# google/dynamic-video-depth

Measured on AMD Instinct MI355X. Metric: train iters/s (depth+sceneflow step) at 384x672, 48 pairs; warp+loss HBM GB/s, higher is better.
Workload: dtype f32 (storage and accumulation fp32; conv / MLP contractions on v_mfma_f32_32x32x16_f16: every fp32 operand, scaled by a power of two from its tensor's max, is split into two fp16 terms (22 bits) and a product is three partial products; <= 4e-6 of max|y| against float64, the bound the 3-term bf16 / 6

## Files before the change

### dynamic-video-depth_amd/dvd_hip/_lib.py

```python
import ctypes
import os
import threading

from . import build as _build

c_float_p = ctypes.c_void_p
c_size_t = ctypes.c_size_t
c_int = ctypes.c_int
c_float = ctypes.c_float
c_void_p = ctypes.c_void_p

DVD_OK, DVD_EINVAL, DVD_EHIP, DVD_ENOSPC = 0, -1, -2, -3
ABI_VERSION = 8


class Cameras(ctypes.Structure):
    _fields_ = [(n, c_void_p) for n in ('R_1', 'R_2', 'R_1_T', 'R_2_T', 't_1', 't_2', 'K', 'K_inv')]


class WarpCfg(ctypes.Structure):
    _fields_ = [('B', c_int), ('H', c_int), ('W', c_int), ('midas_mask', c_int), ('crit_l2', c_int),
                ('disp_mode', c_int), ('loss_on_sf', c_int), ('flow_mul', c_float), ('disp_mul', c_float)]


# ... 60 lines not shown
    'dvd_sf_mlp_gstash_bytes': (c_size_t, [c_longlong]),
    'dvd_sf_mlp_pack': (c_int, [ctypes.POINTER(MlpDesc), ctypes.POINTER(PtrArr6), ctypes.POINTER(PtrArr6), c_void_p,
                                c_void_p]),
    'dvd_sf_mlp_fwd': (c_int, [ctypes.POINTER(MlpDesc), c_void_p, c_void_p, c_void_p, c_float, c_float, c_longlong,
                               c_int, c_void_p, c_void_p, c_void_p, c_void_p, c_void_p]),
    'dvd_sf_mlp_bwd_dx': (c_int, [ctypes.POINTER(MlpDesc), c_void_p, c_void_p, c_float, c_void_p, c_float, c_void_p,
                                  c_void_p, c_void_p, c_longlong, c_int, c_void_p, c_void_p, c_void_p, c_void_p,
                                  c_void_p]),
    'dvd_mul_mask': (c_int, [c_void_p, c_void_p, c_void_p, c_int, c_int, c_longlong, c_void_p]),
    'dvd_scale_add': (c_int, [c_void_p, c_void_p, c_float, c_void_p, c_void_p, c_longlong, c_void_p]),
    'dvd_subsample2_fwd': (c_int, [c_void_p, c_void_p, c_int, c_longlong, c_int, c_int, c_void_p]),
    'dvd_subsample2_bwd': (c_int, [c_void_p, c_void_p, c_int, c_longlong, c_int, c_int, c_void_p]),
    'dvd_avgpool_fwd': (c_int, [c_void_p, c_void_p, c_int, c_longlong] + [c_int] * 5 + [c_void_p]),
    'dvd_avgpool_bwd': (c_int, [c_void_p, c_void_p, c_int, c_longlong] + [c_int] * 5 + [c_void_p]),
    'dvd_depth_tail_fwd': (c_int, [c_void_p, c_void_p, c_longlong, c_void_p]),
    'dvd_depth_tail_bwd': (c_int, [c_void_p, c_void_p, c_void_p, c_longlong, c_void_p]),
    'dvd_acc_reg_workspace_bytes': (c_size_t, []),
    'dvd_acc_reg': (c_int, [c_void_p, c_void_p, c_float, c_void_p, c_void_p, c_void_p, c_int, c_longlong, c_void_p]),
    'dvd_adam_step': (c_int, [c_void_p, c_void_p, c_float, c_void_p, c_void_p, c_void_p, c_void_p, c_longlong, c_float,
                              c_float, c_float, c_float, c_int, c_void_p]),
    'dvd_warp_surfaces': (c_int, [c_void_p, c_void_p, c_void_p, c_void_p, ctypes.POINTER(Cameras),
                                  ctypes.POINTER(Surfaces), c_int, c_int, c_int, c_void_p]),
    'dvd_warp_surfaces_bwd': (c_int, [c_void_p, c_void_p, c_void_p, c_void_p, ctypes.POINTER(Cameras),
                                      ctypes.POINTER(Surfaces), c_void_p, c_void_p, c_void_p, c_int, c_int, c_int, c_void_p]),
    'dvd_flow_warp_fwd': (c_int, [c_void_p, c_void_p, c_void_p, c_int, c_int, c_int, c_int, c_void_p]),
    'dvd_flow_warp_bwd': (c_int, [c_void_p, c_void_p, c_void_p, c_int, c_int, c_int, c_int, c_void_p]),
    'dvd_bnrelu_fwd': (c_int, [c_void_p] * 6 + [c_float, c_void_p, c_int, c_int, c_int, c_int, c_void_p]),
    'dvd_bnrelu_bwd_workspace_bytes': (c_size_t, [c_int, c_int, c_int]),
    'dvd_bnrelu_bwd': (c_int, [c_void_p] * 6 + [c_float] + [c_void_p] * 5 + [c_size_t, c_int, c_int, c_int, c_int,
                                                                           c_void_p, c_void_p]),
    'dvd_upsample_bilinear_fwd': (c_int, [c_void_p, c_void_p, c_longlong, c_int, c_int, c_int, c_int, c_int, c_void_p]),
    'dvd_upsample_bilinear_bwd': (c_int, [c_void_p, c_void_p, c_longlong, c_int, c_int, c_int, c_int, c_int, c_void_p]),
    'dvd_gconv3x3_c8_fwd': (c_int, [c_void_p, c_void_p, c_void_p, c_int, c_int, c_int, c_int, c_void_p]),
    'dvd_gconv3x3_c8_bwd_data': (c_int, [c_void_p, c_void_p, c_void_p, c_int, c_int, c_int, c_int, c_void_p]),
    'dvd_gconv3x3_c8_wgrad_workspace_bytes': (c_size_t, [c_int, c_int, c_int, c_int]),
    'dvd_gconv3x3_c8_bwd_weight': (c_int, [c_void_p, c_void_p, c_void_p, c_int, c_void_p, c_size_t, c_int, c_int, c_int,
                                           c_int, c_void_p]),
    'dvd_gconv3x3_c32_workspace_bytes': (c_size_t, [c_int, c_int, c_int, c_int]),
    'dvd_gconv3x3_c32_fwd': (c_int, [c_void_p, c_void_p, c_void_p, c_void_p, c_size_t, c_int, c_int, c_int, c_int,
                                     c_void_p]),
    'dvd_gconv3x3_c32_bwd_data': (c_int, [c_void_p, c_void_p, c_void_p, c_void_p, c_size_t, c_int, c_int, c_int, c_int,
                                          c_void_p]),
    'dvd_gconv3x3_c32_bwd_weight': (c_int, [c_void_p, c_void_p, c_void_p, c_int, c_void_p, c_size_t, c_int, c_int,
                                            c_int, c_int, c_void_p]),
    'dvd_xconv_packed_bytes': (c_size_t, [c_int] * 5),
    'dvd_xconv_pack': (c_int, [c_void_p, c_void_p, c_int, c_int, c_int, c_int, c_int, c_void_p]),
    'dvd_xconv_pack_table_bytes': (c_size_t, [c_int]),
    'dvd_xconv_pack_many': (c_int, [c_void_p, c_int, c_void_p, c_size_t, c_int, c_void_p]),
    'dvd_amax': (c_int, [c_void_p, ctypes.c_longlong, c_void_p, c_void_p]),
    'dvd_chansum_workspace_bytes': (c_size_t, [c_int, c_int]),
    'dvd_chansum': (c_int, [c_void_p, c_int, c_int, ctypes.c_longlong, c_void_p, c_void_p, c_void_p, c_size_t, c_void_p]),
    'dvd_xconv_fwd': (c_int, [c_void_p] * 6 + [ctypes.POINTER(BnParams), c_void_p, c_void_p] + [c_int] * 8 + [c_void_p]),
    'dvd_xconv_select': (c_int, [c_int]),
    'dvd_xconv_pack_scaled': (c_int, [c_void_p, c_void_p, c_int, c_int, c_int, c_int, c_int, c_void_p, c_void_p, c_float,
                                      c_void_p]),
    'dvd_convbn_finalize': (c_int, [c_void_p] * 6 + [c_float, c_void_p, c_int, c_int, c_void_p, c_void_p, c_void_p]),
    'dvd_xwgrad3_workspace_bytes': (c_size_t, [c_int] * 6),
    'dvd_xwgrad1s_workspace_bytes': (c_size_t, [c_int] * 5),
    'dvd_xwgrad_select': (c_int, [c_int]),
    'dvd_sf_mlp_select': (c_int, [c_int]),
    'dvd_xwgradk_workspace_bytes': (c_size_t, [c_int] * 6),
    'dvd_xwgradk': (c_int, [c_void_p] * 6 + [c_size_t] + [c_int] * 7 + [c_void_p]),
    'dvd_xwgrad1s': (c_int, [c_void_p] * 6 + [c_size_t] + [c_int] * 6 + [c_void_p]),
    'dvd_xwgrad1s_rowsum': (c_int, [c_void_p] * 7 + [c_size_t] + [c_int] * 6 + [c_void_p]),
    'dvd_xwgrad3_rowsum': (c_int, [c_void_p] * 7 + [c_size_t] + [c_int] * 7 + [c_void_p]),
    'dvd_xwgrad_rowsum_in_kernel': (c_int, [c_int] * 7),
    'dvd_xwgrad3': (c_int, [c_void_p] * 6 + [c_size_t] + [c_int] * 7 + [c_void_p]),
    'dvd_xwgrad_workspace_bytes': (c_size_t, [c_int] * 6),
    'dvd_xwgrad': (c_int, [c_void_p] * 4 + [c_size_t] + [c_int] * 7 + [c_void_p]),
    'dvd_flow_consistency_mask': (c_int, [c_void_p, c_void_p, c_void_p, c_int, c_int, c_int, c_void_p]),
    'dvd_sf_mlp_bwd_dw': (c_int, [ctypes.POINTER(MlpDesc), c_void_p, c_void_p, c_longlong, ctypes.POINTER(PtrArr5),
                                  ctypes.POINTER(PtrArr5), c_void_p]),
    'dvd_xconv_fwd_h': (c_int, [c_void_p] * 5 + [ctypes.POINTER(BnParams), c_void_p, c_void_p] + [c_int] * 9 + [c_void_p]),
    'dvd_xwgrad3_h': (c_int, [c_void_p] * 5 + [c_size_t] + [c_int] * 7 + [c_void_p]),
    'dvd_xwgrad1s_h': (c_int, [c_void_p] * 5 + [c_size_t] + [c_int] * 6 + [c_void_p]),
    'dvd_xwgradk_h': (c_int, [c_void_p] * 5 + [c_size_t] + [c_int] * 7 + [c_void_p]),
    'dvd_bnrelu_fwd_t': (c_int, [c_void_p] * 6 + [c_float, c_void_p, c_int, c_int, c_int, c_int, c_int, c_void_p]),
    'dvd_bnrelu_bwd_t': (c_int, [c_void_p] * 6 + [c_float] + [c_void_p] * 5 + [c_size_t, c_int, c_void_p, c_int, c_int, c_int,
                                                                             c_int, c_void_p, c_void_p]),
    'dvd_bnrelu_fwd_m': (c_int, [c_void_p] * 6 + [c_float, c_void_p, c_int, c_int, c_int, c_int, c_int, c_void_p, c_void_p]),
    'dvd_bnrelu_bwd_m': (c_int, [c_void_p] * 6 + [c_float] + [c_void_p] * 5 + [c_size_t, c_int, c_void_p, c_int, c_int, c_int,
                                                                             c_int, c_void_p, c_void_p, c_void_p]),
    'dvd_upsample_bilinear_fwd_t': (c_int, [c_void_p, c_void_p, c_int, c_longlong, c_int, c_int, c_int, c_int, c_int, c_void_p]),
    'dvd_upsample_bilinear_bwd_t': (c_int, [c_void_p, c_void_p, c_int, c_longlong, c_int, c_int, c_int, c_int, c_int, c_void_p]),
    'dvd_bicubic_fwd': (c_int, [c_void_p, c_void_p, c_longlong, c_int, c_int, c_int, c_int, c_void_p, c_void_p, c_int, c_void_p]),
    'dvd_bicubic_bwd_workspace_bytes': (c_size_t, [c_longlong, c_int, c_int, c_int, c_int]),
    'dvd_bicubic_bwd': (c_int, [c_void_p, c_void_p, c_longlong, c_int, c_int, c_int, c_int, c_void_p, c_size_t, c_void_p]),
    'dvd_gconv3x3_c8_fwd_t': (c_int, [c_void_p, c_void_p, c_void_p, c_int, c_int, c_int, c_int, c_int, c_void_p]),
    'dvd_gconv3x3_c8_bwd_data_t': (c_int, [c_void_p, c_void_p, c_void_p, c_int, c_int, c_int, c_int, c_int, c_void_p]),
    'dvd_gconv3x3_c8_bwd_weight_t': (c_int, [c_void_p, c_void_p, c_void_p, c_int, c_void_p, c_size_t, c_int, c_void_p, c_int,
                                             c_int, c_int, c_int, c_void_p]),
    'dvd_head1x1_fwd': (c_int, [c_void_p, c_int, c_void_p, c_void_p, c_void_p, c_void_p, c_int, c_int, c_int, c_int, c_void_p]),
    'dvd_head1x1_bwd_workspace_bytes': (c_size_t, [c_int]),
    'dvd_head1x1_bwd': (c_int, [c_void_p, c_int] + [c_void_p] * 7 + [c_size_t, c_int, c_int, c_int, c_int, c_void_p]),
    'dvd_head3x3_fwd': (c_int, [c_void_p] * 5 + [c_int] * 4 + [c_void_p]),
    'dvd_head3x3_bwd_workspace_bytes': (c_size_t, [c_int] * 4),
    'dvd_head3x3_bwd': (c_int, [c_void_p] * 8 + [c_size_t] + [c_int] * 4 + [c_void_p]),
    'dvd_add_f16': (c_int, [c_void_p] * 3 + [c_longlong, c_void_p, c_void_p]),
    'dvd_gscale_init': (c_int, [c_void_p, c_float, c_void_p]),
    'dvd_gscale_step_begin': (c_int, [c_void_p, c_void_p]),
    'dvd_gscale_begin': (c_int, [c_void_p, c_void_p, c_void_p, c_int, c_void_p]),
    'dvd_gscale_end': (c_int, [c_void_p, c_void_p]),
    'dvd_cast_scale_f32': (c_int, [c_void_p, c_int, c_void_p, c_longlong, c_void_p, c_void_p]),
    'dvd_maxpool3s2_fwd': (c_int, [c_void_p, c_void_p, c_int, c_void_p, c_longlong, c_int, c_int, c_void_p]),
    'dvd_maxpool3s2_bwd': (c_int, [c_void_p, c_int, c_void_p, c_void_p, c_void_p, c_longlong, c_int, c_int, c_void_p]),
    'dvd_adam_step_guarded': (c_int, [c_void_p, c_void_p, c_float, c_void_p, c_void_p, c_void_p, c_void_p, c_longlong, c_float,
# ... 79 lines not shown
```

### dynamic-video-depth_amd/dvd_hip/csrc/xconv.hip

```cpp
#include <type_traits>

#include "dvd_split.h"
#include "xconv_tile.h"

namespace dvd {

typedef float f32x16 __attribute__((ext_vector_type(16)));
typedef float f32x2 __attribute__((ext_vector_type(2)));
typedef unsigned u32x4 __attribute__((ext_vector_type(4)));

#ifndef DVD_XCONV_ROLL
#define DVD_XCONV_ROLL 1
#endif
#ifndef DVD_XCONV_SPARE
#define DVD_XCONV_SPARE 0
#endif
#ifndef DVD_XCONV_DIRECT_BATCH
#define DVD_XCONV_DIRECT_BATCH 4
#endif
constexpr int kXHeader = 16;

__device__ __forceinline__ float xconv_weight(const float* __restrict__ w, int co_g, int idx, const float* __restrict__ sc_gamma,
                                              const float* __restrict__ sc_var, float sc_eps) {
  float val = w[idx];
// ... 868 lines not shown
#pragma unroll
        for (int r = 0; r < 16; ++r) {
          const int co = cob + (r & 3) + 8 * (r >> 2);
          v[r] += a.bias[grp * a.Cout + (co < a.Cout ? co : a.Cout - 1)];
        }
      }
      if (a.bn_var) {
#pragma unroll
        for (int r = 0; r < 16; ++r) {
          const int src = (r & 3) + 8 * (r >> 2) + 4 * (lane >> 5);
          v[r] = __builtin_fmaf(v[r], __shfl(my_sc[tm], src, 64), __shfl(my_sh[tm], src, 64));
        }
      }
      if (a.res) {
        const TY* __restrict__ rb = static_cast<const TY*>(a.res) + ibase;
        float rv[16];
#pragma unroll
        for (int r = 0; r < 16; ++r) {
          const int co = cob + (r & 3) + 8 * (r >> 2);
          rv[r] = (float)rb[(full || co < a.Cout) ? o0 + ((r & 3) + 8 * (r >> 2)) * iplane : pix];
        }
#pragma unroll
        for (int r = 0; r < 16; ++r) v[r] += a.res_relu ? fmaxf(rv[r], 0.0f) : rv[r];
      }
      if (a.mask_src) {
        const TY* __restrict__ mb = static_cast<const TY*>(a.mask_src) + ibase;
        float mv[16];
#pragma unroll
        for (int r = 0; r < 16; ++r) {
          const int co = cob + (r & 3) + 8 * (r >> 2);
          mv[r] = (float)mb[(full || co < a.Cout) ? o0 + ((r & 3) + 8 * (r >> 2)) * iplane : pix];
        }
#pragma unroll
        for (int r = 0; r < 16; ++r) v[r] = mv[r] > 0.0f ? v[r] : 0.0f;
      }
      if (a.relu_out) {
#pragma unroll
        for (int r = 0; r < 16; ++r) v[r] = fmaxf(v[r], 0.0f);
      }
#pragma unroll
      for (int r = 0; r < 16; ++r) {
        const int co = cob + (r & 3) + 8 * (r >> 2);
        if (pok && (full || co < a.Cout)) {
          yb[o0 + ((r & 3) + 8 * (r >> 2)) * iplane] = (TY)v[r];
          ymax = amax_acc(ymax, v[r]);
        }
      }
    }
  }
  if (a.y_amax) wave_amax_to(ymax, a.y_amax);
}

static int g_xcfg = 0;

template <int TM, int TN, int WM, int WN, bool FAST, bool B1 = false, bool IN16 = false, bool OUT16 = false>
static int launch_fi(const XArgs& a, int FI, dim3 grid, size_t lds, hipStream_t s) {
  auto go = [&](auto kern) -> int {
    DVD_HIP_OK(hipFuncSetAttribute(reinterpret_cast<const void*>(kern), hipFuncAttributeMaxDynamicSharedMemorySize, (int)lds));
    hipLaunchKernelGGL(kern, grid, dim3(64 * WM * WN), lds, s, a);
    DVD_LAUNCH_OK();
    return DVD_OK;
  };
  const double flops = 2.0 * a.N * (double)a.G * a.Cout * a.Cin * a.T * (double)a.H * a.W * (a.ZI ? 0.25 : 1.0);
  if constexpr (TM >= 4 && !B1 && FAST && DVD_XCONV_ROLL != 0) {
    if (a.T == 1 && FI == 1 && g_xcfg != 6) {
      flops_add(DVD_FLOP_XCONV_1X1_WIDE, flops);
      return go(xconv_kernel<TM, TN, WM, WN, kXFitOne, FAST, B1, IN16, OUT16>);
    }
  }
  flops_add(TM >= 4 ? DVD_FLOP_XCONV_WIDE : (WM == 2 ? DVD_FLOP_XCONV_128 : DVD_FLOP_XCONV_SMALL), flops);
  switch (FI) {
    case 1: return go(xconv_kernel<TM, TN, WM, WN, 1, FAST, B1, IN16, OUT16>);
    case 2: return go(xconv_kernel<TM, TN, WM, WN, 2, FAST, B1, IN16, OUT16>);
    case 3: return go(xconv_kernel<TM, TN, WM, WN, 3, FAST, B1, IN16, OUT16>);
    default: return go(xconv_kernel<TM, TN, WM, WN, 0, FAST, B1, IN16, OUT16>);
  }
}

static int xconv_mtiles(int M) {
  const int bm = M <= 32 ? 32 : (M <= 64 ? 64 : (M >= 256 ? 256 : 128));
  return (M + bm - 1) / bm * (bm / 32);
}

}

extern "C" {

size_t dvd_xconv_packed_bytes(int Cout, int Cin, int KS, int groups, int transposed) {
  if (Cout <= 0 || Cin <= 0 || KS <= 0 || !(KS & 1) || groups <= 0 || Cout % groups || Cin % groups) return 0;
  const int co = Cout / groups, ci = Cin / groups;
  const int M = transposed ? ci : co, K = transposed ? co : ci;
  return ((size_t)dvd::kXHeader + (size_t)groups * dvd::xconv_mtiles(M) * ((K + 15) / 16) * KS * KS * 2 * 64) * sizeof(uint4);
}

static int xconv_pack_impl(const float* w, void* packed, int Cout, int Cin, int KS, int groups, int transposed,
                           const float* gamma, const float* var, float eps, dvd_stream_t stream) {
  DVD_REQUIRE(w && packed, "xconv_pack: null pointer");
  DVD_REQUIRE(Cout > 0 && Cin > 0 && KS > 0 && (KS & 1) && KS <= 11 && groups > 0 && Cout % groups == 0 && Cin % groups == 0,
              "xconv_pack: bad shape Cout=%d Cin=%d KS=%d groups=%d", Cout, Cin, KS, groups);
  const int co = Cout / groups, ci = Cin / groups;
  const int M = transposed ? ci : co, K = transposed ? co : ci;
  const int mtiles = dvd::xconv_mtiles(M), nkc = (K + 15) / 16, T = KS * KS;
  const long long total = (long long)groups * mtiles * nkc * T * 64;
  dvd::bytes_add(DVD_BYTES_PACK, 8.0 * (double)Cout * ci * T + 16.0 * (double)total);
  const int row_len = ci * T;
  int npart;
// ... 31 lines not shown

int dvd_xconv_pack_many(const dvd_xpack_item* items, int n, void* table, size_t table_bytes, int upload, dvd_stream_t stream) {
  DVD_REQUIRE(items && table && n > 0, "xconv_pack_many: bad arguments");
  DVD_REQUIRE(table_bytes >= dvd_xconv_pack_table_bytes(n), "xconv_pack_many: table %zu < %zu bytes", table_bytes,
              dvd_xconv_pack_table_bytes(n));
  std::vector<dvd::XPackDev> host((size_t)n);
  unsigned long long blocks = 0;
  double bytes = 0.0;
  for (int i = 0; i < n; ++i) {
    const dvd_xpack_item& q = items[i];
    DVD_REQUIRE(q.w && q.packed, "xconv_pack_many: item %d: null pointer", i);
    DVD_REQUIRE(q.Cout > 0 && q.Cin > 0 && q.KS > 0 && (q.KS & 1) && q.KS <= 11 && q.groups > 0 && q.Cout % q.groups == 0 &&
                    q.Cin % q.groups == 0,
                "xconv_pack_many: item %d: bad shape Cout=%d Cin=%d KS=%d groups=%d", i, q.Cout, q.Cin, q.KS, q.groups);
    DVD_REQUIRE(!q.gamma || q.var, "xconv_pack_many: item %d: BatchNorm scale without a variance", i);
    dvd::XPackDev& d = host[(size_t)i];
    d.w = q.w;
    d.packed = static_cast<uint4*>(q.packed);
    d.gamma = q.gamma;
    d.var = q.var;
    d.eps = q.eps;
    d.co = q.Cout / q.groups;
    d.ci = q.Cin / q.groups;
    d.T = q.KS * q.KS;
    d.transposed = q.transposed ? 1 : 0;
    const int M = d.transposed ? d.ci : d.co, K = d.transposed ? d.co : d.ci;
    d.mtiles = dvd::xconv_mtiles(M);
    d.nkc = (K + 15) / 16;
    d.G = q.groups;
    d.rows = q.Cout;
    d.row_len = d.ci * d.T;
    d.block0 = (unsigned)blocks;
    d.pad_ = 0;
    const long long total = (long long)d.G * d.mtiles * d.nkc * d.T * 64;
    blocks += (unsigned long long)((total + 255) / 256);
    bytes += 8.0 * (double)q.Cout * d.ci * d.T + 16.0 * (double)total;
  }
  DVD_REQUIRE(blocks < (1ull << 31), "xconv_pack_many: too many blocks");
  hipStream_t st = static_cast<hipStream_t>(stream);
  if (upload) {
    DVD_HIP_OK(hipMemcpyAsync(table, host.data(), (size_t)n * sizeof(dvd::XPackDev), hipMemcpyHostToDevice, st));
    DVD_HIP_OK(hipStreamSynchronize(st));
  }
  dvd::bytes_add(DVD_BYTES_PACK, bytes);
  const dvd::XPackDev* t = static_cast<const dvd::XPackDev*>(table);
  hipLaunchKernelGGL(dvd::xconv_wamax_many_kernel, dim3(dvd::kManyPartials, (unsigned)n), dim3(64 * dvd::kWamaxWaves), 0, st, t);
  DVD_LAUNCH_OK();
  hipLaunchKernelGGL(dvd::xconv_pack_many_kernel, dim3((unsigned)blocks), dim3(256), 0, st, t, n);
  DVD_LAUNCH_OK();
  return DVD_OK;
}

int dvd_xconv_select(int cfg) {
  DVD_REQUIRE(cfg >= 0 && cfg <= dvd::kXSelHalo, "xconv_select: cfg %d", cfg);
  dvd::g_xcfg = cfg;
  return DVD_OK;
}

static int xconv_fwd_impl(const void* x, const float* x_amax, const void* packed, const float* bias, const void* residual,
                          const void* mask_src, const dvd_bn_params* bn, void* y, float* y_amax, int N, int Cin_total,
                          int Cout_total, int H, int W, int KS, int groups, int flags, int in16, int out16, dvd_stream_t stream) {
  DVD_REQUIRE(x && packed && y, "xconv: null pointer");
  DVD_REQUIRE(in16 || x_amax, "xconv: the input's max|x| scalar is missing (dvd_amax, or the producer's y_amax)");
  DVD_REQUIRE(N > 0 && Cin_total > 0 && Cout_total > 0 && H > 0 && W > 0, "xconv: bad shape N=%d Cin=%d Cout=%d H=%d W=%d", N,
              Cin_total, Cout_total, H, W);
  DVD_REQUIRE(groups > 0 && Cin_total % groups == 0 && Cout_total % groups == 0, "xconv: %d groups do not divide the channels",
              groups);
  DVD_REQUIRE(KS > 0 && (KS & 1) && KS <= 11, "xconv: kernel size %d (odd sizes up to 11)", KS);
  DVD_REQUIRE(N <= 65535, "xconv: too many images for the grid");
  DVD_REQUIRE((long long)H * W * (long long)(Cin_total > Cout_total ? Cin_total : Cout_total) < (1ll << 31),
              "xconv: image too large for 32-bit offsets");
  DVD_REQUIRE(in16 || !out16, "xconv: fp32 input with fp16 output is not a configuration of this kernel");
  const int s2 = (flags >> 3) & 1, zi = (flags >> 4) & 1;
  DVD_REQUIRE(!(s2 && zi), "xconv: stride-2 forward and stride-2 backward-data are different launches");
  DVD_REQUIRE(!(s2 || zi) || KS == 3, "xconv: the strided forms exist for 3x3 kernels (got %d)", KS);
  const int Hq = (H + 1) / 2, Wq = (W + 1) / 2;
  const int Cin = Cin_total / groups, Cout = Cout_total / groups;
  dvd::XPlan plan;
  const bool planned = dvd::xconv_plan(Cin, Cout, H, W, KS, s2 != 0, in16 != 0, dvd::g_xcfg, plan);
  const bool fast = plan.fast;
  DVD_REQUIRE(fast || !in16, "xconv: fp16 activations need input channels in multiples of 16 (got %d per group)", Cin);
  DVD_REQUIRE(!(s2 || zi) || fast, "xconv: the strided forms need input channels in multiples of 16 (got %d per group)", Cin);
  DVD_REQUIRE(planned, "xconv: no %stile of a %dx%d image with a %dx%d kernel fits the LDS", s2 ? "stride-2 " : "", H, W, KS, KS);
  const dvd::XCfg& c = plan.c;
  const dvd::XTile& t = plan.t;
  const int Hh = plan.Hh, Ww = plan.Ww, S2 = plan.S2;
  dvd::XArgs a;
  a.x = x;
  a.wp = static_cast<const uint4*>(packed);
  a.bias = bias;
  a.res = residual;
  a.mask_src = mask_src;
  a.bn_gamma = bn ? bn->gamma : nullptr;
  a.bn_beta = bn ? bn->beta : nullptr;
  a.bn_mean = bn ? bn->mean : nullptr;
  a.bn_var = bn ? bn->var : nullptr;
  a.bn_eps = bn ? bn->eps : 0.0f;
  DVD_REQUIRE(!bn || (bn->mean && bn->var), "xconv: BatchNorm statistics missing");
  a.y = y;
  a.x_amax = x_amax;
  a.y_amax = y_amax;
  a.N = N; a.Cin = Cin; a.Cout = Cout; a.H = Hh; a.W = Ww;
  a.G = groups; a.mtiles = dvd::xconv_mtiles(Cout);
  a.KS = KS; a.pad = KS / 2; a.T = KS * KS;
  a.TR = t.TR; a.TC = t.TC; a.P = t.P; a.PQ = t.PQ; a.ntr = t.ntr; a.ntc = t.ntc; a.NV = t.NV;
  a.nkc = (Cin + 15) / 16; a.npos = t.npos; a.nfi = t.FI;
  a.Hi = s2 ? H : (zi ? Hq : Hh); a.Wi = s2 ? W : (zi ? Wq : Ww); a.S2 = S2; a.ZI = zi;
  a.relu_in = flags & 1; a.relu_out = (flags >> 1) & 1; a.res_relu = (flags >> 2) & 1;
  const int mblocks = plan.mblocks;
  a.mbpg = mblocks;
  DVD_REQUIRE((long long)mblocks * groups <= 65535, "xconv: too many channel blocks");
  const dim3 grid(t.ntr * t.ntc, mblocks * groups, N);
  auto al16 = [](const void* p) { return (reinterpret_cast<uintptr_t>(p) & 15) == 0; };
  a.vec_out = (KS == 1 && ((long long)H * W) % 8 == 0 && t.TC % 8 == 0 && al16(y) && al16(residual) && al16(mask_src) &&
               dvd::g_xcfg != 7) ? 1 : 0;
  size_t lds = t.lds;
  if (a.vec_out && lds < (size_t)c.NT() / 64 * 32 * 68 * 4) lds = (size_t)c.NT() / 64 * 32 * 68 * 4;
  hipStream_t s = static_cast<hipStream_t>(stream);
#define DVD_XGO(TM_, TN_, WM_, WN_)                                                                                      \
  do {                                                                                                                   \
    if (in16 && out16) return dvd::launch_fi<TM_, TN_, WM_, WN_, true, false, true, true>(a, t.FI, grid, lds, s);         \
    if (in16) return dvd::launch_fi<TM_, TN_, WM_, WN_, true, false, true, false>(a, t.FI, grid, lds, s);                 \
    return dvd::launch_fi<TM_, TN_, WM_, WN_, true>(a, t.FI, grid, lds, s);                                               \
  } while (0)
  if (fast) {
    if (c.TM == 4 && c.WN == 4) DVD_XGO(4, 2, 2, 4);
    if (c.TM == 4) DVD_XGO(4, 2, 2, 2);
    if (c.WM == 2 && c.b1) return dvd::launch_fi<2, 2, 2, 2, true, true>(a, t.FI, grid, lds, s);
    if (c.TM == 2 && c.WM == 1 && c.b1) return dvd::launch_fi<2, 2, 1, 4, true, true>(a, t.FI, grid, lds, s);
    if (c.TM == 1 && c.b1) return dvd::launch_fi<1, 2, 1, 4, true, true>(a, t.FI, grid, lds, s);
    if (c.WM == 2) DVD_XGO(2, 2, 2, 2);
    if (c.TM == 2) DVD_XGO(2, 2, 1, 4);
// ... 24 lines not shown
```

### dynamic-video-depth_amd/dvd_hip/csrc/xconv_tile.h

```cpp
#pragma once
#include <cstddef>

#if defined(__HIPCC__) || defined(__CUDACC__)
#define DVD_XTILE_HD __host__ __device__
#else
#define DVD_XTILE_HD
#endif

namespace dvd {

DVD_XTILE_HD inline int xconv_cell(int q, int PQ, int P, int TR) {
  const int rr = q / PQ;
  return rr < TR ? rr * P + (q - rr * PQ) : 0;
}
DVD_XTILE_HD inline int xconv_tapoff(int ky, int kx, int P, int S2) {
  return S2 ? ((ky & 1) * 2 + (kx & 1)) * S2 + (ky >> 1) * P + (kx >> 1) : ky * P + kx;
}

struct XCfg {
  int TM, TN, WM, WN;
  bool b1 = false;
  bool in16 = false;
  int blockM() const { return TM * WM * 32; }
  int NQ() const { return TN * WN * 32; }
  int NT() const { return 64 * WM * WN; }
};
constexpr int kXSelHalo = 8;
inline XCfg pick_cfg(int M, int KS, int sel) {
  if (M <= 32) return {1, 2, 1, 4};
  if (M <= 64) return {2, 2, 1, 4};
  if (M > 64 && sel == 5) return {2, 2, 2, 2, true};
  if (M >= 256 && sel != 1 && sel != 4) {
    if (sel == 2) return {4, 2, 2, 2};
    if (sel == 3) return {4, 2, 2, 4};
    return KS == 1 ? XCfg{4, 2, 2, 2} : XCfg{4, 2, 2, 4};
  }
  return {2, 2, 2, 2};
}
constexpr int kXLdsBudget = 78 * 1024;
constexpr int kXLdsBudgetOne = 156 * 1024;
constexpr int kXLdsBudgetB1 = 52 * 1024;
constexpr int kXMaxFI = 3;
constexpr int kXMaxFIDirect = 16;

struct XTile {
  int TR, TC, P, PQ, ntr, ntc, NV, npos, FI;
  size_t lds;
};
inline size_t xconv_lds(const XCfg& c, int npos) {
  const int AU = c.WM * c.TM * 128, NT = c.NT();
  const int AS = (AU + NT - 1) / NT * NT;
  return ((size_t)2 * AS + (size_t)(c.b1 ? 4 : 8) * npos / (c.in16 ? 2 : 1)) * 16;
}
inline bool pick_tile_halo_budget(int H, int W, int KS, const XCfg& c, XTile& best, int budget) {
  const int pad = KS / 2, NQ = c.NQ(), NT = c.NT();
  double best_eff = -1.0;
  for (int nct = 1; nct <= W; ++nct) {
    int TC = (W + nct - 1) / nct;
    if (KS == 1) TC = (TC + 7) & ~7;
    const int P = TC + 2 * pad;
    if (P > NQ) continue;
    const int ntc = (W + TC - 1) / TC;
    const int npos = NQ + (KS - 1) * (P + 1) + 1;
    if (xconv_lds(c, npos) > (size_t)budget) continue;
    int trmax = NQ / P;
    if (trmax > H) trmax = H;
    for (int tr0 = trmax; tr0 >= 1; --tr0) {
      const int ntr = (H + tr0 - 1) / tr0;
      const int TR = (H + ntr - 1) / ntr;
      const int NV = (TR + 2 * pad) * P;
      const int FI = (2 * NV + NT - 1) / NT;
      if (FI > kXMaxFIDirect) continue;
      const double eff = (double)H * W / ((double)ntr * ntc * NQ) - 0.02 * (double)NV / (TR * TC) - 1e-6 * nct;
      if (eff > best_eff) {
        best_eff = eff;
        best = {TR, TC, P, P, ntr, ntc, NV, npos, FI, xconv_lds(c, npos)};
      }
      break;
    }
    if (TC <= 8) break;
  }
  return best_eff > -1.0;
}
// ... 71 lines not shown
    const int ntc = (Wo + TC - 1) / TC;
    int trmax = NQ / PQ;
    if (trmax > Ho) trmax = Ho;
    const int ntr = (Ho + trmax - 1) / trmax;
    const int TR = (Ho + ntr - 1) / ntr;
    const int s2 = (TR + 1) * P;
    const int npos = 3 * s2 + (halo ? NQ : TR * P) + 1;
    const int NV = (2 * TR + 1) * (2 * TC + 1);
    const int FI = (2 * NV + NT - 1) / NT;
    if (xconv_lds(c, npos) <= (size_t)budget && FI <= 4 * kXMaxFIDirect) {
      const double eff = (double)Ho * Wo / ((double)ntr * ntc * NQ) - 1e-6 * nct;
      if (eff > best_eff) {
        best_eff = eff;
        best = {TR, TC, P, PQ, ntr, ntc, NV, npos, FI, xconv_lds(c, npos)};
        S2 = s2;
      }
    }
    if (TC <= 4) break;
  }
  return best_eff > -1.0;
}
inline bool pick_tile_s2(int Ho, int Wo, const XCfg& c, XTile& best, int& S2, bool halo) {
  const int budgets[2] = {kXLdsBudget, kXLdsBudgetOne};
  for (int budget : budgets) {
    XTile h;
    int sh = 0;
    if (!pick_tile_s2_budget(Ho, Wo, c, h, sh, budget, true)) continue;
    best = h;
    S2 = sh;
    if (halo) return true;
    XTile d;
    int sd = 0;
    const int tier = h.lds <= (size_t)kXLdsBudgetB1 ? kXLdsBudgetB1 : budget;
    if (pick_tile_s2_budget(Ho, Wo, c, d, sd, tier, false) && d.ntr * d.ntc <= h.ntr * h.ntc) {
      best = d;
      S2 = sd;
    } else {
      best.PQ = h.TC;
      best.npos = 3 * sh + h.TR * h.P + 1;
      best.lds = xconv_lds(c, best.npos);
    }
    return true;
  }
  return false;
}

struct XPlan {
  XCfg c;
  XTile t;
  int S2;
  int Hh, Ww;
  bool fast;
  int mblocks;
};
inline bool xconv_plan(int Cin, int Cout, int H, int W, int KS, bool s2, bool in16, int sel, XPlan& p) {
  p.fast = (Cin % 16 == 0) && ((long long)Cin * H * W * 4 < (1ll << 31)) &&
           ((long long)8 * ((Cin + 15) / 16) * KS * KS * 2048 < (1ll << 31)) && sel != 4;
  p.c = pick_cfg((p.fast && !s2) ? Cout : (Cout < 128 ? Cout : 128), KS, sel);
  if (!p.fast) p.c.b1 = false;
  if (s2) p.c.b1 = true;
  if (in16) p.c.b1 = false;
  p.c.in16 = in16;
  p.Hh = H;
  p.Ww = W;
  if (KS == 1) {
    p.Hh = 1;
    p.Ww = H * W;
  }
  p.S2 = 0;
  const bool halo = sel == kXSelHalo || xconv_keeps_halo_positions(Cin, Cout, H, W, KS, s2);
  bool ok;
  if (s2) {
    p.Hh = (H + 1) / 2;
    p.Ww = (W + 1) / 2;
    ok = pick_tile_s2(p.Hh, p.Ww, p.c, p.t, p.S2, halo);
  } else {
    if (p.c.b1 && !pick_tile(p.Hh, p.Ww, KS, p.c, p.t, halo)) p.c.b1 = false;
    ok = pick_tile(p.Hh, p.Ww, KS, p.c, p.t, halo);
  }
  p.mblocks = (Cout + p.c.blockM() - 1) / p.c.blockM();
  return ok;
}

}
```

### dynamic-video-depth_amd/dvd_hip/ops.py

```python
import ctypes
import os
import sys

import numpy as np
import torch

from . import _lib

CAM_KEYS = ('R_1', 'R_2', 'R_1_T', 'R_2_T', 't_1', 't_2', 'K', 'K_inv')


def _p(t):
    return ctypes.c_void_p(t.data_ptr()) if t is not None else ctypes.c_void_p(0)


def _stream():
    return ctypes.c_void_p(torch.cuda.current_stream().cuda_stream)


def _dev32(t, name):
    if not (torch.is_tensor(t) and t.is_cuda):
        raise RuntimeError('%s must be a GPU tensor (dvd_hip has no CPU path)' % name)
    if t.dtype != torch.float32:
        raise RuntimeError('%s must be float32, got %s' % (name, t.dtype))
# ... 1053 lines not shown
        out = torch.empty((U_pad,) + tuple(g_d1.shape[1:]), device=g_d1.device, dtype=torch.float32)
    elif _union_rows('union_reduce', out, U_pad, 'out', torch.float32) != bpr:
        raise RuntimeError('union_reduce: out must hold %d rows like the sources\'' % U_pad)
    _lib.check(_lib.load().dvd_union_reduce(_p(g_d1), _p(g_d2), _p(out), _p(tab.part('offsets')), _p(tab.part('entries')), U_pad,
                                            B, bpr // 4, _stream()), 'dvd_union_reduce')
    return out


class _BicubicResize(torch.autograd.Function):
    @staticmethod
    def forward(ctx, x, size, mean, std):
        N, C, H, W = x.shape
        Ho, Wo = size
        y = torch.empty(N, C, Ho, Wo, device=x.device, dtype=torch.float32)
        _lib.check(_lib.load().dvd_bicubic_fwd(_p(x), _p(y), N * C, H, W, Ho, Wo, _p(mean), _p(std), C, _stream()), 'dvd_bicubic_fwd')
        ctx.shape = (N, C, H, W, Ho, Wo)
        return y

    @staticmethod
    def backward(ctx, gy):
        N, C, H, W, Ho, Wo = ctx.shape
        gy = _dev32(gy, 'gy')
        lib = _lib.load()
        gx = torch.empty(N, C, H, W, device=gy.device, dtype=torch.float32)
        ws = torch.empty(max(1, lib.dvd_bicubic_bwd_workspace_bytes(N * C, H, W, Ho, Wo)), device=gy.device, dtype=torch.uint8)
        _lib.check(lib.dvd_bicubic_bwd(_p(gy), _p(gx), N * C, H, W, Ho, Wo, _p(ws), ws.numel(), _stream()), 'dvd_bicubic_bwd')
        return gx, None, None, None


def bicubic_resize(x, size, mean=None, std=None):
    x = _dev32(x, 'x')
    if x.dim() != 4 or x.numel() == 0:
        raise RuntimeError('bicubic_resize: x must be a non-empty [N,C,H,W] tensor, got shape %s' % (tuple(x.shape),))
    Ho, Wo = (int(v) for v in size)
    if Ho <= 0 or Wo <= 0:
        raise RuntimeError('bicubic_resize: size must be positive, got %s' % ((Ho, Wo),))
    if (mean is None) != (std is None):
        raise RuntimeError('bicubic_resize: mean and std go together')
    if mean is not None:
        mean, std = _dev32(mean, 'mean'), _dev32(std, 'std')
        if mean.numel() != x.shape[1] or std.numel() != x.shape[1] or mean.device != x.device or std.device != x.device:
            raise RuntimeError('bicubic_resize: mean / std must hold one value per channel (%d) on the device of x' % x.shape[1])
        if x.requires_grad:
            raise RuntimeError('bicubic_resize: the normalising form has no backward (x must not require a gradient)')
    return _BicubicResize.apply(x, (Ho, Wo), mean, std)


def warp_loss_select(variant='tiled', tile=-1, px=0, strip_rows=0, strip_shape=0):
    lib = _lib.load()
    _lib.check(lib.dvd_warp_loss_select({'tiled': 0, 'direct': 1, 'tiles': 2}[variant], int(tile), int(px)), 'dvd_warp_loss_select')
    _lib.check(lib.dvd_warp_loss_strip_select(int(strip_rows), int(strip_shape)), 'dvd_warp_loss_strip_select')


def loss_finalize(cfg, sums, out=None):
    sums = _dev32(sums, 'sums')
    if out is None:
        out = torch.empty(8, device=sums.device, dtype=torch.float32)
    lib = _lib.load()
    _lib.check(lib.dvd_loss_finalize(ctypes.byref(cfg), _p(sums), _p(out), _stream()), 'dvd_loss_finalize')
    return out


_SURFACE_SHAPES = {'global_p1': 3, 'warped_global_p2': 3, 'sf_by_depth': 3, 'p1_camera_2': 3, 'warped_p2_camera_2': 3,
                   'staticflow_1_2': 2, 'dflow_1_2': 2, 'depth_image_1_2': 1, 'depth_warp_1_2': 1}


def warp_surfaces(depth_1, depth_2, flow_1_2, cams, sflow_1_2=None, want=_lib.SURFACE_KEYS):
    depth_1, depth_2, flow_1_2 = _dev32(depth_1, 'depth_1'), _dev32(depth_2, 'depth_2'), _dev32(flow_1_2, 'flow_1_2')
    B, _, H, W = depth_1.shape
    if sflow_1_2 is not None:
        sflow_1_2 = _dev32(sflow_1_2, 'sflow_1_2')
        if sflow_1_2.numel() != 3 * B * H * W:
            raise RuntimeError('sflow_1_2 must be [B,H,W,1,3]')
    cst, keep = pack_cameras(cams)
    out, st = {}, _lib.Surfaces()
    for k in want:
        c = _SURFACE_SHAPES[k]
        shape = (B, H, W, 1, 3) if c == 3 else ((B, H, W, 2) if c == 2 else (B, 1, H, W))
        out[k] = torch.empty(shape, device=depth_1.device, dtype=torch.float32)
        setattr(st, k, out[k].data_ptr())
    lib = _lib.load()
    _lib.check(lib.dvd_warp_surfaces(_p(depth_1), _p(depth_2), _p(flow_1_2), _p(sflow_1_2), ctypes.byref(cst),
                                     ctypes.byref(st), B, H, W, _stream()), 'dvd_warp_surfaces')
    del keep
    return out


def warp_surfaces_backward(depth_1, depth_2, flow_1_2, cams, grads, sflow_1_2=None, want_sflow_grad=False):
    depth_1, depth_2, flow_1_2 = _dev32(depth_1, 'depth_1'), _dev32(depth_2, 'depth_2'), _dev32(flow_1_2, 'flow_1_2')
    B, _, H, W = depth_1.shape
    if sflow_1_2 is not None:
        sflow_1_2 = _dev32(sflow_1_2, 'sflow_1_2')
    cst, keep = pack_cameras(cams)
    st = _lib.Surfaces()
    for k in _lib.SURFACE_KEYS:
        g = grads.get(k)
        if g is not None:
            g = _dev32(g, 'grad of ' + k)
            if g.numel() != _SURFACE_SHAPES[k] * B * H * W:
                raise RuntimeError('gradient of %s has the wrong size' % k)
            keep.append(g)
            setattr(st, k, g.data_ptr())
    g1, g2 = torch.empty_like(depth_1), torch.empty_like(depth_2)
    gs = torch.empty(B, H, W, 1, 3, device=depth_1.device, dtype=torch.float32) if want_sflow_grad else None
    _lib.check(_lib.load().dvd_warp_surfaces_bwd(_p(depth_1), _p(depth_2), _p(flow_1_2), _p(sflow_1_2), ctypes.byref(cst),
                                                 ctypes.byref(st), _p(g1), _p(g2), _p(gs), B, H, W, _stream()),
# ... 178 lines not shown
```

### include/dvd_hip.h

```cpp
#ifndef DVD_HIP_H
#define DVD_HIP_H

#include <stddef.h>
#include <stdint.h>

#ifdef __cplusplus
extern "C" {
#endif

#define DVD_ABI_VERSION 8

typedef void* dvd_stream_t;

typedef enum dvd_status {
  DVD_OK = 0,
  DVD_EINVAL = -1,
  DVD_EHIP = -2,
  DVD_ENOSPC = -3
} dvd_status;

int dvd_abi_version(void);
const char* dvd_last_error(void);
int dvd_device_cu_count(void);

// ... 146 lines not shown
                           dvd_stream_t stream);
int dvd_gconv3x3_c8_bn_bwd_data(const float* g, const float* w, const float* gamma, const float* var, float eps,
                                const float* mask_src, float* gx, float* gx_amax, int N, int C, int H, int W,
                                dvd_stream_t stream);
size_t dvd_gconv3x3_c8_bn_wgrad_workspace_bytes(int N, int C, int H, int W);
int dvd_gconv3x3_c8_bn_bwd_weight(const float* x, const float* g, float* gw, float* g_chansum, void* workspace,
                                  size_t workspace_bytes, int N, int C, int H, int W, dvd_stream_t stream);

size_t dvd_gconv3x3_c32_workspace_bytes(int N, int C, int H, int W);
int dvd_gconv3x3_c32_fwd(const float* x, const float* w, float* y, void* workspace, size_t workspace_bytes, int N,
                         int C, int H, int W, dvd_stream_t stream);
int dvd_gconv3x3_c32_bwd_data(const float* gy, const float* w, float* gx, void* workspace, size_t workspace_bytes,
                              int N, int C, int H, int W, dvd_stream_t stream);
int dvd_gconv3x3_c32_bwd_weight(const float* x, const float* gy, float* gw, int accumulate, void* workspace,
                                size_t workspace_bytes, int N, int C, int H, int W, dvd_stream_t stream);

int dvd_bnrelu_fwd(const float* x, const float* residual, const float* gamma, const float* beta, const float* mean,
                   const float* var, float eps, float* y, int N, int C, int HW, int relu, dvd_stream_t stream);
size_t dvd_bnrelu_bwd_workspace_bytes(int N, int C, int HW);
int dvd_bnrelu_bwd(const float* gy, const float* y, const float* x, const float* gamma, const float* mean,
                   const float* var, float eps, float* gx, float* g_residual, float* g_gamma, float* g_beta,
                   void* workspace, size_t workspace_bytes, int N, int C, int HW, int relu, float* g_amax, dvd_stream_t stream);

int dvd_upsample_bilinear_fwd(const float* x, float* y, long long planes, int H_in, int W_in, int H_out, int W_out,
                              int align_corners, dvd_stream_t stream);
int dvd_upsample_bilinear_bwd(const float* gy, float* gx, long long planes, int H_in, int W_in, int H_out,
                              int W_out, int align_corners, dvd_stream_t stream);

int dvd_bicubic_fwd(const float* x, float* y, long long planes, int H_in, int W_in, int H_out, int W_out, const float* mean,
                    const float* std, int channels, dvd_stream_t stream);
size_t dvd_bicubic_bwd_workspace_bytes(long long planes, int H_in, int W_in, int H_out, int W_out);
int dvd_bicubic_bwd(const float* gy, float* gx, long long planes, int H_in, int W_in, int H_out, int W_out, void* workspace,
                    size_t workspace_bytes, dvd_stream_t stream);

int dvd_amax(const float* x, long long n, float* out, dvd_stream_t stream);

size_t dvd_chansum_workspace_bytes(int N, int C);
int dvd_chansum(const float* x, int N, int C, long long HW, float* out, float* amax_out, void* workspace, size_t workspace_bytes,
                dvd_stream_t stream);

size_t dvd_xconv_packed_bytes(int Cout, int Cin, int KS, int groups, int transposed);
int dvd_xconv_pack(const float* w, void* packed, int Cout, int Cin, int KS, int groups, int transposed, dvd_stream_t stream);
typedef struct dvd_bn_params {
  const float* gamma;
  const float* beta;
  const float* mean;
  const float* var;
  float eps;
} dvd_bn_params;
int dvd_xconv_fwd(const float* x, const float* x_amax, const void* packed, const float* bias, const float* residual,
                  const float* mask_src, const dvd_bn_params* bn, float* y, float* y_amax, int N, int Cin, int Cout, int H,
                  int W, int KS, int groups, int flags, dvd_stream_t stream);
int dvd_xconv_select(int cfg);
int dvd_xconv_pack_scaled(const float* w, void* packed, int Cout, int Cin, int KS, int groups, int transposed,
                          const float* bn_gamma, const float* bn_var, float bn_eps, dvd_stream_t stream);
typedef struct dvd_xpack_item {
  const float* w;
  void* packed;
  const float* gamma;
  const float* var;
  float eps;
  int Cout, Cin, KS, groups, transposed;
} dvd_xpack_item;
size_t dvd_xconv_pack_table_bytes(int n);
int dvd_xconv_pack_many(const dvd_xpack_item* items, int n, void* table, size_t table_bytes, int upload, dvd_stream_t stream);
int dvd_convbn_finalize(const float* W, float* dW, const float* dbeta, const float* gamma, const float* mean, const float* var,
                        float eps, const float* conv_bias, int Cout, int K, float* dgamma, float* dconv_bias, dvd_stream_t stream);
size_t dvd_xwgrad_workspace_bytes(int N, int Cin, int Cout, int H, int W, int KS);
int dvd_xwgrad(const float* x, const float* gy, float* gw, void* workspace, size_t workspace_bytes, int N, int Cin,
               int Cout, int H, int W, int KS, int relu_in, dvd_stream_t stream);

size_t dvd_xwgrad3_workspace_bytes(int N, int Cin, int Cout, int H, int W, int groups);
int dvd_xwgrad3(const float* x, const float* x_amax, const float* gy, const float* gy_amax, float* gw, void* workspace,
                size_t workspace_bytes, int N, int Cin, int Cout, int H, int W, int groups, int relu_in, dvd_stream_t stream);
size_t dvd_xwgrad1s_workspace_bytes(int N, int Cin, int Cout, int H, int W);
int dvd_xwgrad1s(const float* x, const float* x_amax, const float* gy, const float* gy_amax, float* gw, void* workspace,
                 size_t workspace_bytes, int N, int Cin, int Cout, int H, int W, int relu_in, dvd_stream_t stream);
int dvd_xwgrad1s_rowsum(const float* x, const float* x_amax, const float* gy, const float* gy_amax, float* gw, float* gy_rowsum,
                        void* workspace, size_t workspace_bytes, int N, int Cin, int Cout, int H, int W, int relu_in,
                        dvd_stream_t stream);
int dvd_xwgrad3_rowsum(const float* x, const float* x_amax, const float* gy, const float* gy_amax, float* gw, float* gy_rowsum,
                       void* workspace, size_t workspace_bytes, int N, int Cin, int Cout, int H, int W, int groups, int relu_in,
                       dvd_stream_t stream);
int dvd_xwgrad_rowsum_in_kernel(int N, int Cin, int Cout, int H, int W, int KS, int groups);
int dvd_xwgrad_select(int variant);
size_t dvd_xwgradk_workspace_bytes(int N, int Cin, int Cout, int H, int W, int KS);
int dvd_xwgradk(const float* x, const float* x_amax, const float* gy, const float* gy_amax, float* gw, void* workspace,
                size_t workspace_bytes, int N, int Cin, int Cout, int H, int W, int KS, int relu_in, dvd_stream_t stream);

int dvd_flow_consistency_mask(const float* flow_a, const float* flow_b, float* mask, int B, int H, int W,
                              dvd_stream_t stream);

int dvd_xconv_fwd_h(const void* x, const void* packed, const float* bias, const void* residual, const void* mask_src,
                    const dvd_bn_params* bn, void* y, float* y_amax, int N, int Cin_total, int Cout_total, int H, int W, int KS,
                    int groups, int flags, int out_f16, dvd_stream_t stream);
int dvd_xwgrad3_h(const void* x, const void* gy, const float* out_scale, float* gw, void* workspace, size_t workspace_bytes, int N,
                  int Cin_total, int Cout_total, int H, int W, int groups, int relu_in, dvd_stream_t stream);
int dvd_xwgrad1s_h(const void* x, const void* gy, const float* out_scale, float* gw, void* workspace, size_t workspace_bytes, int N,
                   int Cin, int Cout, int H, int W, int relu_in, dvd_stream_t stream);
int dvd_xwgradk_h(const void* x, const void* gy, const float* out_scale, float* gw, void* workspace, size_t workspace_bytes, int N,
                  int Cin, int Cout, int H, int W, int KS, int relu_in, dvd_stream_t stream);
int dvd_bnrelu_fwd_t(const void* x, const void* residual, const float* gamma, const float* beta, const float* mean,
                     const float* var, float eps, void* y, int f16, int N, int C, int HW, int relu, dvd_stream_t stream);
int dvd_bnrelu_bwd_t(const void* gy, const void* y, const void* x, const float* gamma, const float* mean, const float* var,
                     float eps, void* gx, void* g_residual, float* g_gamma, float* g_beta, void* workspace,
                     size_t workspace_bytes, int f16, const float* out_scale, int N, int C, int HW, int relu, float* g_amax,
// ... 139 lines not shown
```

Baseline: 1.689.

## Pick xconv tile config by modelled CU fill when the grid is small or ragged

```diff
diff --git a/dynamic-video-depth_amd/dvd_hip/_lib.py b/dynamic-video-depth_amd/dvd_hip/_lib.py
--- a/dynamic-video-depth_amd/dvd_hip/_lib.py
+++ b/dynamic-video-depth_amd/dvd_hip/_lib.py
@@ -136,6 +136,8 @@
     'dvd_chansum': (c_int, [c_void_p, c_int, c_int, ctypes.c_longlong, c_void_p, c_void_p, c_void_p, c_size_t, c_void_p]),
     'dvd_xconv_fwd': (c_int, [c_void_p] * 6 + [ctypes.POINTER(BnParams), c_void_p, c_void_p] + [c_int] * 8 + [c_void_p]),
     'dvd_xconv_select': (c_int, [c_int]),
+    'dvd_xconv_plan_cus': (c_int, [c_int]),
+    'dvd_xconv_plan_info': (c_int, [c_int] * 10 + [ctypes.POINTER(c_longlong), c_int]),
     'dvd_xconv_pack_scaled': (c_int, [c_void_p, c_void_p, c_int, c_int, c_int, c_int, c_int, c_void_p, c_void_p, c_float,
                                       c_void_p]),
     'dvd_convbn_finalize': (c_int, [c_void_p] * 6 + [c_float, c_void_p, c_int, c_int, c_void_p, c_void_p, c_void_p]),
diff --git a/dynamic-video-depth_amd/dvd_hip/csrc/xconv.hip b/dynamic-video-depth_amd/dvd_hip/csrc/xconv.hip
--- a/dynamic-video-depth_amd/dvd_hip/csrc/xconv.hip
+++ b/dynamic-video-depth_amd/dvd_hip/csrc/xconv.hip
@@ -944,6 +944,18 @@
 }
 
 static int g_xcfg = 0;
+static int g_xcus = 0;
+
+static int xconv_cus() {
+  if (g_xcus > 0) return g_xcus;
+  static int cached[64] = {};
+  int dev = 0, n = 0;
+  if (hipGetDevice(&dev) != hipSuccess || dev < 0 || dev >= 64) return 0;
+  if (cached[dev] > 0) return cached[dev];
+  if (hipDeviceGetAttribute(&n, hipDeviceAttributeMultiprocessorCount, dev) != hipSuccess || n <= 0) return 0;
+  cached[dev] = n;
+  return n;
+}
 
 template <int TM, int TN, int WM, int WN, bool FAST, bool B1 = false, bool IN16 = false, bool OUT16 = false>
 static int launch_fi(const XArgs& a, int FI, dim3 grid, size_t lds, hipStream_t s) {
@@ -1081,8 +1093,33 @@
 }
 
 int dvd_xconv_select(int cfg) {
-  DVD_REQUIRE(cfg >= 0 && cfg <= dvd::kXSelHalo, "xconv_select: cfg %d", cfg);
+  DVD_REQUIRE(cfg >= 0 && cfg <= dvd::kXSelMax, "xconv_select: cfg %d", cfg);
   dvd::g_xcfg = cfg;
+  return DVD_OK;
+}
+
+int dvd_xconv_plan_cus(int cus) {
+  DVD_REQUIRE(cus >= 0, "xconv_plan_cus: %d CUs", cus);
+  dvd::g_xcus = cus;
+  return DVD_OK;
+}
+
+int dvd_xconv_plan_info(int N, int Cin_total, int Cout_total, int H, int W, int KS, int groups, int s2, int in16, int cus,
+                        long long* out, int n) {
+  DVD_REQUIRE(out && n >= DVD_XPLAN_FIELDS, "xconv_plan_info: room for %d values", DVD_XPLAN_FIELDS);
+  DVD_REQUIRE(N > 0 && Cin_total > 0 && Cout_total > 0 && H > 0 && W > 0 && KS > 0 && (KS & 1) && KS <= 11 && groups > 0 &&
+                  Cin_total % groups == 0 && Cout_total % groups == 0,
+              "xconv_plan_info: bad shape N=%d Cin=%d Cout=%d H=%d W=%d KS=%d groups=%d", N, Cin_total, Cout_total, H, W, KS, groups);
+  if (cus == 0) cus = dvd::xconv_cus();
+  DVD_REQUIRE(cus != 0, "xconv_plan_info: no device to take the CU count from");
+  dvd::XPlan p;
+  const int Cin = Cin_total / groups, Cout = Cout_total / groups;
+  const bool ok = cus < 0 ? dvd::xconv_plan(Cin, Cout, H, W, KS, s2 != 0, in16 != 0, dvd::g_xcfg, p)
+                          : dvd::xconv_plan(Cin, Cout, H, W, KS, s2 != 0, in16 != 0, dvd::g_xcfg, (long long)N * groups, cus, p);
+  DVD_REQUIRE(ok, "xconv_plan_info: no tile of a %dx%d image with a %dx%d kernel fits the LDS", H, W, KS, KS);
+  const long long v[DVD_XPLAN_FIELDS] = {p.c.TM, p.c.TN, p.c.WM, p.c.WN, p.c.b1, p.t.TR, p.t.TC, p.t.ntr, p.t.ntc, p.mblocks,
+                                         p.t.FI, (long long)p.t.lds, p.per_cu, p.blocks, p.refit, p.fast};
+  for (int i = 0; i < DVD_XPLAN_FIELDS; ++i) out[i] = v[i];
   return DVD_OK;
 }
 
@@ -1106,7 +1143,7 @@
   const int Hq = (H + 1) / 2, Wq = (W + 1) / 2;
   const int Cin = Cin_total / groups, Cout = Cout_total / groups;
   dvd::XPlan plan;
-  const bool planned = dvd::xconv_plan(Cin, Cout, H, W, KS, s2 != 0, in16 != 0, dvd::g_xcfg, plan);
+  const bool planned = dvd::xconv_plan(Cin, Cout, H, W, KS, s2 != 0, in16 != 0, dvd::g_xcfg, (long long)N * groups, dvd::xconv_cus(), plan);
   const bool fast = plan.fast;
   DVD_REQUIRE(fast || !in16, "xconv: fp16 activations need input channels in multiples of 16 (got %d per group)", Cin);
   DVD_REQUIRE(!(s2 || zi) || fast, "xconv: the strided forms need input channels in multiples of 16 (got %d per group)", Cin);
diff --git a/dynamic-video-depth_amd/dvd_hip/csrc/xconv_tile.h b/dynamic-video-depth_amd/dvd_hip/csrc/xconv_tile.h
--- a/dynamic-video-depth_amd/dvd_hip/csrc/xconv_tile.h
+++ b/dynamic-video-depth_amd/dvd_hip/csrc/xconv_tile.h
@@ -26,9 +26,12 @@
   int NT() const { return 64 * WM * WN; }
 };
 constexpr int kXSelHalo = 8;
+constexpr int kXSel64 = 9;
+constexpr int kXSel32 = 10;
+constexpr int kXSelMax = 10;
 inline XCfg pick_cfg(int M, int KS, int sel) {
-  if (M <= 32) return {1, 2, 1, 4};
-  if (M <= 64) return {2, 2, 1, 4};
+  if (M <= 32 || sel == kXSel32) return {1, 2, 1, 4};
+  if (M <= 64 || sel == kXSel64) return {2, 2, 1, 4};
   if (M > 64 && sel == 5) return {2, 2, 2, 2, true};
   if (M >= 256 && sel != 1 && sel != 4) {
     if (sel == 2) return {4, 2, 2, 2};
@@ -206,11 +209,14 @@
   int Hh, Ww;
   bool fast;
   int mblocks;
+  int per_cu = 0;
+  long long blocks = 0;
+  double rounds = 0.0;
+  bool refit = false;
 };
-inline bool xconv_plan(int Cin, int Cout, int H, int W, int KS, bool s2, bool in16, int sel, XPlan& p) {
-  p.fast = (Cin % 16 == 0) && ((long long)Cin * H * W * 4 < (1ll << 31)) &&
-           ((long long)8 * ((Cin + 15) / 16) * KS * KS * 2048 < (1ll << 31)) && sel != 4;
-  p.c = pick_cfg((p.fast && !s2) ? Cout : (Cout < 128 ? Cout : 128), KS, sel);
+inline bool xconv_plan_shape(const XCfg& c, bool fast, int Cout, int H, int W, int KS, bool s2, bool in16, bool halo, XPlan& p) {
+  p.fast = fast;
+  p.c = c;
   if (!p.fast) p.c.b1 = false;
   if (s2) p.c.b1 = true;
   if (in16) p.c.b1 = false;
@@ -222,7 +228,6 @@
     p.Ww = H * W;
   }
   p.S2 = 0;
-  const bool halo = sel == kXSelHalo || xconv_keeps_halo_positions(Cin, Cout, H, W, KS, s2);
   bool ok;
   if (s2) {
     p.Hh = (H + 1) / 2;
@@ -233,7 +238,72 @@
     ok = pick_tile(p.Hh, p.Ww, KS, p.c, p.t, halo);
   }
   p.mblocks = (Cout + p.c.blockM() - 1) / p.c.blockM();
+  p.per_cu = 0;
+  p.blocks = 0;
+  p.rounds = 0.0;
+  p.refit = false;
   return ok;
 }
-
-}
+inline bool xconv_fast(int Cin, int H, int W, int KS, int sel) {
+  return (Cin % 16 == 0) && ((long long)Cin * H * W * 4 < (1ll << 31)) &&
+         ((long long)8 * ((Cin + 15) / 16) * KS * KS * 2048 < (1ll << 31)) && sel != 4;
+}
+inline bool xconv_plan(int Cin, int Cout, int H, int W, int KS, bool s2, bool in16, int sel, XPlan& p) {
+  const bool fast = xconv_fast(Cin, H, W, KS, sel);
+  const XCfg c = pick_cfg((fast && !s2) ? Cout : (Cout < 128 ? Cout : 128), KS, sel);
+  const bool halo = sel == kXSelHalo || xconv_keeps_halo_positions(Cin, Cout, H, W, KS, s2);
+  return xconv_plan_shape(c, fast, Cout, H, W, KS, s2, in16, halo, p);
+}
+
+constexpr double kXFillFewRounds = 3.0;
+constexpr double kXFillMfma = 0.2;
+constexpr double kXFillStage = 0.084;
+constexpr double kXFillStage16 = 0.126;
+constexpr double kXFillLone = 0.4;
+constexpr double kXFillMargin = 0.07;
+inline int xconv_blocks_per_cu(const XCfg& c, size_t lds) {
+  if (c.NT() >= 512) return 1;
+  if (c.b1 && lds <= (size_t)kXLdsBudgetB1) return 3;
+  return lds <= (size_t)kXLdsBudget ? 2 : 1;
+}
+inline double xconv_fill(XPlan& p, int Cin, int KS, long long nimg, int cus) {
+  const XCfg& c = p.c;
+  p.per_cu = xconv_blocks_per_cu(c, p.t.lds);
+  p.blocks = (long long)p.t.ntr * p.t.ntc * p.mblocks * nimg;
+  p.rounds = (double)p.blocks / ((double)p.per_cu * cus);
+  const long long on_cu = (p.blocks + cus - 1) / cus;
+  const int wps = c.NT() / 256;
+  const double ksteps = (double)((Cin + 15) / 16) * KS * KS;
+  const double mfmas = (c.in16 ? 4.0 : 6.0) * c.TM * c.TN, reads = c.in16 ? 2.0 * c.TM + c.TN : 3.0 * (c.TM + c.TN);
+  const double per_mfma = kXFillMfma + reads / mfmas + (c.in16 ? kXFillStage16 : kXFillStage) * 288.0 / ((double)c.blockM() * KS * KS);
+  const double lone = (on_cu < p.per_cu ? on_cu : p.per_cu) * wps == 1 ? 1.0 + kXFillLone : 1.0;
+  return (double)on_cu * lone * wps * mfmas * ksteps * per_mfma;
+}
+inline bool xconv_plan(int Cin, int Cout, int H, int W, int KS, bool s2, bool in16, int sel, long long nimg, int cus, XPlan& p) {
+  if (!xconv_plan(Cin, Cout, H, W, KS, s2, in16, sel, p)) return false;
+  if (cus <= 0 || nimg <= 0) return true;
+  double best = xconv_fill(p, Cin, KS, nimg, cus);
+  if (sel != 0 || s2 || !p.fast || Cout <= 64) return true;
+  const bool under = p.blocks < (long long)p.per_cu * cus;
+  const bool ragged = p.rounds < kXFillFewRounds && p.blocks % ((long long)p.per_cu * cus) != 0;
+  if (!under && !ragged) return true;
+  const bool halo = xconv_keeps_halo_positions(Cin, Cout, H, W, KS, s2);
+  const XCfg cands[5] = {{4, 2, 2, 2}, {2, 2, 2, 2}, {2, 2, 2, 2, true}, {2, 2, 1, 4}, {1, 2, 1, 4}};
+  const double need = best * (1.0 - kXFillMargin);
+  for (const XCfg& c : cands) {
+    if (c.TM == 4 && (KS == 1 || Cout < 256)) continue;
+    if (c.b1 && in16) continue;
+    if (c.TM == p.c.TM && c.WM == p.c.WM && c.WN == p.c.WN && c.b1 == p.c.b1) continue;
+    XPlan q;
+    if (!xconv_plan_shape(c, true, Cout, H, W, KS, false, in16, halo, q) || q.c.b1 != c.b1) continue;
+    const double cost = xconv_fill(q, Cin, KS, nimg, cus);
+    if (cost < need && cost < best) {
+      best = cost;
+      p = q;
+      p.refit = true;
+    }
+  }
+  return true;
+}
+
+}
diff --git a/dynamic-video-depth_amd/dvd_hip/ops.py b/dynamic-video-depth_amd/dvd_hip/ops.py
--- a/dynamic-video-depth_amd/dvd_hip/ops.py
+++ b/dynamic-video-depth_amd/dvd_hip/ops.py
@@ -1129,6 +1129,24 @@
     _lib.check(lib.dvd_warp_loss_strip_select(int(strip_rows), int(strip_shape)), 'dvd_warp_loss_strip_select')
 
 
+XPLAN_FIELDS = ('TM', 'TN', 'WM', 'WN', 'b1', 'TR', 'TC', 'ntr', 'ntc', 'mblocks', 'FI', 'lds', 'per_cu', 'blocks', 'refit', 'fast')
+
+
+def xconv_plan_cus(cus=0):
+    _lib.check(_lib.load().dvd_xconv_plan_cus(int(cus)), 'dvd_xconv_plan_cus')
+
+
+def xconv_plan(N, Cin, Cout, H, W, KS, groups=1, s2=False, in16=False, cus=0):
+    out = (_lib.c_longlong * len(XPLAN_FIELDS))()
+    _lib.check(_lib.load().dvd_xconv_plan_info(int(N), int(Cin), int(Cout), int(H), int(W), int(KS), int(groups), int(bool(s2)),
+                                               int(bool(in16)), int(cus), out, len(XPLAN_FIELDS)), 'dvd_xconv_plan_info')
+    p = dict(zip(XPLAN_FIELDS, (int(v) for v in out)))
+    p['shape'] = (32 * p['TM'] * p['WM'], 32 * p['TN'] * p['WN'])
+    if cus > 0:
+        p['rounds'] = p['blocks'] / (p['per_cu'] * cus)
+    return p
+
+
 def loss_finalize(cfg, sums, out=None):
     sums = _dev32(sums, 'sums')
     if out is None:
diff --git a/include/dvd_hip.h b/include/dvd_hip.h
--- a/include/dvd_hip.h
+++ b/include/dvd_hip.h
@@ -222,6 +222,10 @@
                   const float* mask_src, const dvd_bn_params* bn, float* y, float* y_amax, int N, int Cin, int Cout, int H,
                   int W, int KS, int groups, int flags, dvd_stream_t stream);
 int dvd_xconv_select(int cfg);
+int dvd_xconv_plan_cus(int cus);
+#define DVD_XPLAN_FIELDS 16
+int dvd_xconv_plan_info(int N, int Cin, int Cout, int H, int W, int KS, int groups, int s2, int in16, int cus, long long* out,
+                        int n);
 int dvd_xconv_pack_scaled(const float* w, void* packed, int Cout, int Cin, int KS, int groups, int transposed,
                           const float* bn_gamma, const float* bn_var, float bn_eps, dvd_stream_t stream);
 typedef struct dvd_xpack_item {
```

After: 1.698, median of 6. No clear change (+0.5%).
